# degleris1/CMF.jl

Hardware: AMD Instinct MI355X
Metric: MU iters/sec (convolutive NMF multiplicative update; achieved HBM GB/s in `hbm`) (higher is better)
Workload: dtype f32

## Files before the change

cmf.jl_amd/csrc/cmf_api.hip:

```cpp
#include "cmf_internal.h"

static void wb_free(cmf_handle_s *h);
static void wb_disarm(cmf_handle_s *h);

size_t n_partial(const cmf_handle_s *h)
{
    const CmfDims &d = h->d;
    size_t n = (size_t)(64 * h->conv_gx) * (size_t)std::max(h->conv_gy, h->conv_gy_ext);
    n = std::max(n, (size_t)(d.Np / 64) * d.KB * d.L);
    n = std::max(n, (size_t)((d.Tl + 63) / 64) * d.KB);
    n = std::max(n, 2 * (((size_t)d.Tl * d.K32 + 1023) / 1024));
    return n;
}

static int ensure_stage(cmf_handle_s *h, size_t elems)
{
    if (h->stage_elems >= elems) return CMF_OK;
    if (h->stage) HIPCHK(hipFree(h->stage));
    h->stage = nullptr;
    h->stage_elems = 0;
    HIPCHK(hipMalloc(&h->stage, elems * sizeof(double)));
    h->stage_elems = elems;
    return CMF_OK;
}
// ... 342 lines not shown
        TRYB(upload_cols(h, data, 0, Tl, true, true));
        if (h->halo_r > 0) TRYB(upload_cols(h, data + (size_t)Tl * N, Tl, h->halo_r, false, false));
        h->data_norm = std::sqrt(h->data_sumsq);
        h->have_data = true;
    }
#undef TRYB
#undef HIPB
    *out = h;
    return CMF_OK;
}


int launch_hxt_on(cmf_handle_s *h, const float *X0, const float *X1, int NpX, int nsrc, float *slabs, int nchunks, int chunk_len,
                         int main_rows, const float *left)
{
    ProfScope prof_(h, hxt_prof_class(h, X0, nsrc));
    const CmfDims &d = h->d;
    h->spec_gen = -1;
    HxtParams p;
    p.H = left ? left : h->H; p.X0 = X0; p.X1 = X1; p.slabs = slabs;
    p.Np = NpX; p.K32 = d.K32; p.KB = d.KB; p.PADL = d.PADL; p.L = d.L; p.Tl = main_rows >= 0 ? main_rows : d.Tl; p.chunk_len = chunk_len;
    p.G = h->hxt_groups; p.nsrc = nsrc;
    p.CG = hxt_cg(nchunks);
    dim3 grid((NpX / 128) * p.CG * h->hxt_groups, nchunks / p.CG, nsrc * d.KB), block(256);
    switch (h->hxt_LP) {
#define CASE(LP_) case LP_: hipLaunchKernelGGL((hxt_kernel<LP_>), grid, block, 0, h->stream, p); break;
        CASE(1) CASE(2) CASE(3) CASE(4) CASE(5) CASE(6) CASE(8)
#undef CASE
    default: return fail(CMF_ERR_STATE, "internal: bad hxt LP %d", h->hxt_LP);
    }
    for (int i = 0; i < 7; ++i)
        if (kHxtLP[i] == h->hxt_LP) h->launches[LA_HXT + i] += 1;
    h->launches[nsrc == 1 ? LA_HXT_NSRC1 : LA_HXT_NSRC2] += 1;
    h->launches[p.Tl < d.Tl ? LA_HXT_TAIL : LA_HXT_NO_TAIL] += 1;
    KCHK("hxt_kernel");
    return CMF_OK;
}

int launch_transconv(cmf_handle_s *h, int nsrc, const float *xt0, bool front_block)
{
    if (h->sk_tc) return launch_transconv_small(h, nsrc, xt0);
    ProfScope prof_(h, nsrc == 2 ? PROF_TRANSCONV : PROF_TRANSCONV_1);
    const CmfDims &d = h->d;
    TcParams p;
    p.Wn = h->Wn; p.XT0 = xt0 ? xt0 : h->XT; p.XT1 = h->estT; p.slabs = h->hslabs;
    p.NpW = d.Np;
    p.TP = d.TP; p.PADL = d.PADL; p.K32 = d.K32; p.KB = d.KB; p.L = d.L; p.Tl = d.Tl;
    p.nsrc = nsrc;
    p.C = (int)(rup(d.N, 8) / 8);
    p.W = nsrc == 2 ? h->tc_W : h->tc_W1;
    p.F = nsrc == 2 ? h->tc_S : h->tc_S1;
    p.wtab = h->tc_tab[nsrc == 2 ? 0 : 1];
    p.t_first = 0;
    p.slab_rows = d.Tl;
    if (front_block) {
        p.W = h->tc_W2; p.F = h->tc_S2; p.wtab = h->tc_tab[2];
        p.t_first = -128;
        p.slab_rows = d.Tl + 128;
// ... 9 lines not shown
    if (front_block) h->launches[LA_TC_FRONT] += 1;
    if (p.W >= 64 && p.W % 32 == 0) h->launches[LA_TC_XCD] += 1;
    KCHK("transconv_kernel");
    return CMF_OK;
}

int launch_slab_sum(cmf_handle_s *h, float *out, const float *in, int nslabs, size_t stride, bool take_carry,
                           CmfHxtTail tail)
{
    size_t n4 = stride / 4;
    int blocks = (int)std::min<size_t>(2048, (n4 + 255) / 256);
    CmfLossCarry carry{};
    if (take_carry && h->carry.partial) {
        carry = h->carry;
        h->carry = CmfLossCarry{};
    }
    hipLaunchKernelGGL(slab_sum_kernel, dim3(blocks + (carry.partial ? 1 : 0)), dim3(256), 0, h->stream, out, in, nslabs, stride, n4, carry, tail);
    h->launches[carry.partial ? LA_SLAB_SUM_CARRY : LA_SLAB_SUM] += 1;
    KCHK("slab_sum_kernel");
    return CMF_OK;
}

int hxt_contract(cmf_handle_s *h, const float *X0, const float *X1, int nsrc, float *out, bool take_carry, bool slabs_only, const float *left,
                 const float *leftT)
{
    const CmfDims &d = h->d;
    h->spec_gen = -1;
    if ((left == nullptr) != (leftT == nullptr)) return fail(CMF_ERR_STATE, "internal: a left operand of the C2 contraction needs both layouts");
    if (h->small_k) return hxt_contract_small(h, X0, X1, nsrc, out, take_carry, slabs_only, leftT);
    const int nch = nsrc == 2 ? h->hxt_nchunks : h->hxt_nchunks1, clen = nsrc == 2 ? h->hxt_chunk_len : h->hxt_chunk_len1;
    const int main_rows = nsrc == 2 ? h->hxt_main : h->hxt_main1;
    CMFTRY(launch_hxt_on(h, X0, X1, d.Np, nsrc, h->wslabs, nch, clen, main_rows, left));
    const CmfHxtTail tail{left ? left : h->H, X0, X1, d.Tl - main_rows, d.PADL + main_rows, d.L, d.K32, d.Np};
    return launch_slab_sum(h, out, h->wslabs, hxt_nslabs(nch), (size_t)nsrc * d.L * d.K32 * d.Np, take_carry, tail);
}

int read_scalar(cmf_handle_s *h, int slot, double *v)
{
    HIPCHK(hipMemcpyAsync(h->h_scalar + slot, h->d_scalar + slot, sizeof(double), hipMemcpyDeviceToHost, h->stream));
    HIPCHK(hipStreamSynchronize(h->stream));
    *v = h->h_scalar[slot];
    return CMF_OK;
}

static int check_ready(cmf_handle_s *h, bool need_data)
{
    if (!h) return fail(CMF_ERR_ARG, "handle is NULL");
    if (h->root_only) return fail(CMF_ERR_STATE, "this entry needs a single-GPU handle, not the front handle of a cmf_create_multi group");
    HIPCHK(hipSetDevice(h->device));
    if (!h->factors_set) return fail(CMF_ERR_STATE, "factors not set: call cmf_set_factors first");
    if (need_data && !h->have_data) return fail(CMF_ERR_STATE, "handle was created without data");
    return CMF_OK;
}

[[maybe_unused]] static void conv_kernel_order()
{
// ... 17 lines not shown
        CASE(CONV_ISM_PQ) CASE(CONV_ISM_PQ_T) CASE(CONV_ISM_LOSS) CASE(CONV_ISM_LOSS_PQ)
        CASE(CONV_BETAM_PQ) CASE(CONV_BETAM_PQ_T) CASE(CONV_BETAM_LOSS) CASE(CONV_BETAM_LOSS_PQ)
#undef CASE
    default: return fail(CMF_ERR_STATE, "internal: the MU rule launches no conv mode %d", conv_mode(family, base));
    }
}

static int mu_conv(cmf_handle_s *h, int base, float *out, int T_store, int gy)
{
    const MuForm &f = mu_form(h);
    return mu_launch_conv(h, base >= CONV_BASE_LOSS ? f.loss_family : f.store_family, base, out, T_store, gy, mu_buf(h, f.conv_data[base]));
}

static bool mu_est_current(const cmf_handle_s *h) { return h->reuse_est && h->est_kind == mu_est_kind(h); }

static bool w_speculated(cmf_handle_s *h)
{
    const bool hit = mu_fusions(h) && h->spec_gen >= 0 && h->spec_gen == h->est_gen && mu_est_current(h) && !h->carry.partial;
    h->spec_gen = -1;
    if (hit) h->spec_hits += 1;
    return hit;
}

static int mu_contract_c2(cmf_handle_s *h, bool slabs_only)
{
    const MuForm &f = mu_form(h);
    return hxt_contract(h, mu_buf(h, f.c2_src[0]), mu_buf(h, f.c2_src[1]), f.c2_nsrc, slabs_only ? nullptr : h->numden, !slabs_only, slabs_only);
}

static int mu_contract_w(cmf_handle_s *h, bool slabs_only)
{
    if (w_speculated(h)) return CMF_OK;
    if (!mu_est_current(h)) CMFTRY(mu_conv(h, CONV_BASE_STORE, h->est, h->d.Tl, h->conv_gy));
    set_est(h, mu_est_kind(h));
    return mu_contract_c2(h, slabs_only);
}

int w_partial_impl(cmf_handle_s *h) { return mu_contract_w(h, false); }

int w_partial_half_impl(cmf_handle_s *h, int den)
{
    const CmfDims &d = h->d;
    const size_t LKN = (size_t)d.L * d.K32 * d.Np;
    if (den) {
        if (!(h->reuse_est && h->est_kind == EST_CONV))
            CMFTRY(launch_conv<CONV_EST>(h, h->est, d.Tl, h->conv_gy));
        set_est(h, EST_CONV);
    }
    const float *src = den ? h->est : h->X;
    return hxt_contract(h, src, src, 1, h->numden + (den ? LKN : 0), den != 0);
}

int w_apply_impl(cmf_handle_s *h, double l1W, double l2W, const float *tail_src, float *tail_dst, int tail_n, const float *den)
{
    const CmfDims &d = h->d;
    dim3 grid(d.Np / 64, d.KB, d.L);
    if (!den) den = h->numden + (size_t)d.L * d.K32 * d.Np;
    const int step = mu_step_kind(h, mu_form(h));
    if (step == 2) {
        hipLaunchKernelGGL(w_update_pow_kernel, grid, dim3(256), 0, h->stream, h->Wt, h->Wn, h->numden, den, d.N, d.K, d.L, d.Np, d.K32, (float)l1W,
                           (float)(2.0 * l2W), tail_src, tail_dst, tail_n, h->mu_gamma);
        KCHK("w_update_pow_kernel");
        h->pow_launches += 1;
        set_est(h, EST_NONE);
        return CMF_OK;
    }
    const bool root = step == 1;
    hipLaunchKernelGGL(root ? w_update_sqrt_kernel : w_update_kernel, grid, dim3(256), 0, h->stream, h->Wt, h->Wn, h->numden, den,
                       d.N, d.K, d.L, d.Np, d.K32, (float)l1W, (float)(2.0 * l2W), tail_src, tail_dst, tail_n);
    KCHK(root ? "w_update_sqrt_kernel" : "w_update_kernel");
    set_est(h, EST_NONE);
    return CMF_OK;
}

static int w_phase_impl(cmf_handle_s *h, double l1W, double l2W)
{
    const CmfDims &d = h->d;
    const MuForm &f = mu_form(h);
    if (!(h->small_k && mu_fusions(h))) {
        CMFTRY(w_partial_impl(h));
        if (f.kl_den()) {
            hipLaunchKernelGGL(kl_hsum_kernel, dim3(d.K, KL_HCHUNKS), dim3(256), 0, h->stream, h->Ht, d.TP, d.PADL, d.Tl, h->kl_sums);
            KCHK("kl_hsum_kernel");
            hipLaunchKernelGGL(kl_den_w_kernel, dim3(d.L, d.K), dim3(256), 0, h->stream, h->Ht, h->kl_sums, h->numden + (size_t)d.L * d.K32 * d.Np, d.TP, d.PADL, d.Tl,
                               d.K32, d.Np);
            KCHK("kl_den_w_kernel");
        }
        if (!xo_active(h)) return w_apply_impl(h, l1W, l2W);
        CMFTRY(xo_fold_w(h));
        CMFTRY(w_apply_impl(h, l1W, l2W));
        xo_after_w(h);
        return CMF_OK;
    }
    CMFTRY(mu_contract_w(h, true));
    CmfLossCarry carry{};
    if (h->carry.partial) {
        carry = h->carry;
        h->carry = CmfLossCarry{};
    }
    hipLaunchKernelGGL(w_update_small_kernel, dim3(d.Np / 64 + 1, d.L, d.K), dim3(256), 0, h->stream, h->Wt, h->Wn, h->sk_tc ? h->sk_Wj : nullptr, h->sk_slabs,
                       h->sk_ngroups, d.N, d.K, d.L, d.Np, d.K32, h->sk_JP, h->sk3_Kg, h->sk3_GR, h->sk3_JP,
                       (float)l1W, (float)(2.0 * l2W), carry);
// ... 54 lines not shown
        KCHK("kl_den_h_kernel");
    }
    const int S = f.c3_nsrc == 2 ? h->tc_S : h->tc_S1;
    if (xo_active(h)) {
        const float *num = nullptr, *den = nullptr;
        CMFTRY(xo_h_tables(h, S, stride, f.h_num, f.h_den, &num, &den));
        return launch_h_update(h, mu_step_kind(h, f), num, (size_t)0, 1, den, (size_t)0, 1, d.Tl, d.PADL, l1H, l2H);
    }
    if (f.kl_den()) return launch_h_update(h, mu_step_kind(h, f), h->hslabs + f.h_num * TK, stride, S, h->kl_denH, (size_t)0, 1, d.Tl, d.PADL, l1H, l2H);
    return launch_h_update(h, mu_step_kind(h, f), h->hslabs + f.h_num * TK, stride, S, h->hslabs + f.h_den * TK, stride, S, d.Tl, d.PADL, l1H, l2H);
}

int launch_loss_conv(cmf_handle_s *h)
{
    if (!(h->reuse_est && !h->gram)) return mu_conv(h, CONV_BASE_LOSS, nullptr, h->d.Tl, h->conv_gy);
    CMFTRY(mu_conv(h, CONV_BASE_LOSS_STORE, h->est, h->d.Tl, h->conv_gy));
    set_est(h, mu_est_kind(h));
    return CMF_OK;
}

static int w_speculate(cmf_handle_s *h)
{
    if (!mu_est_current(h) || h->gram || h->group || h->carry.partial || !mu_fusions(h)) return CMF_OK;
    CMFTRY(mu_contract_c2(h, h->small_k));
    h->spec_gen = h->est_gen;
    return CMF_OK;
}

static int ensure_ring(cmf_handle_s *h)
{
    if (!h->h_ring) HIPCHK(hipHostMalloc(&h->h_ring, 3 * sizeof(double), hipHostMallocCoherent));
    return CMF_OK;
}

int loss_partial_impl(cmf_handle_s *h, double *sumsq, bool readback, double *host_out, bool speculate)
{
    volatile unsigned long long *word = nullptr;
    if (readback && !host_out) {
        CMFTRY(ensure_ring(h));
        host_out = h->h_ring + 2;
        word = reinterpret_cast<volatile unsigned long long *>(host_out);
        *word = CMF_SENTINEL64;
    }
    CMFTRY(launch_loss_conv(h));
    hipLaunchKernelGGL(loss_reduce_kernel, dim3(1), dim3(256), 0, h->stream, h->partial, h->conv_partials, h->d_scalar, host_out);
    KCHK("loss_reduce_kernel");
    if (speculate) CMFTRY(w_speculate(h));
// ... 423 lines not shown
}

int cmf_rccl_version(int *version, char *path, int64_t path_len)
{
    if (!version) return fail(CMF_ERR_ARG, "version is NULL");
    CMFTRY(rccl_load());
    RCCLCHK(g_rccl.GetVersion(version));
    if (path && path_len > 0) snprintf(path, (size_t)path_len, "%s", g_rccl.path.c_str());
    return CMF_OK;
}

int cmf_get_counter(cmf_handle h, const char *name, int64_t *value)
{
    if (!h || !name || !value) return fail(CMF_ERR_ARG, "NULL argument");
    if (std::strcmp(name, "hals_pipeline_reruns") == 0) { *value = h->hals_reruns; return CMF_OK; }
    if (std::strcmp(name, "plan:n_cu") == 0) {
        *value = (h->root_only && h->group && !h->group->sh.empty()) ? h->group->sh[0]->n_cu : h->n_cu;
        return CMF_OK;
    }
    if (std::strcmp(name, "writeback_calls") == 0) { *value = h->wb ? h->wb->armed_calls : 0; return CMF_OK; }
    if (std::strcmp(name, "speculated_contractions") == 0) { *value = h->spec_hits; return CMF_OK; }
    if (std::strcmp(name, "liveness_checks") == 0) { *value = g_liveness_checks.load(); return CMF_OK; }
    if (std::strcmp(name, "pow_update_launches") == 0) { *value = h->pow_launches; return CMF_OK; }
    if (std::strcmp(name, "xortho_launches") == 0) { *value = h->xo_launches; return CMF_OK; }
    if (admm_counter(h, name, value)) return CMF_OK;
    if (sep_counter(h, name, value)) return CMF_OK;
    if (anls_counter(h, name, value)) return CMF_OK;
    if (std::strcmp(name, "small_k_fused_h_updates") == 0) {
        *value = h->sk_fused_h;
        if (h->group)
            for (const cmf_handle_s *s : h->group->sh) *value += (s != h) ? s->sk_fused_h : 0;
        return CMF_OK;
    }
    if (std::strcmp(name, "writeback_overlapped") == 0) { *value = h->wb ? h->wb->hooked_calls : 0; return CMF_OK; }
    if (std::strncmp(name, "launches:", 9) == 0) {
        for (int c = 0; c < LA_NCLS; ++c)
            if (std::strcmp(name + 9, kLaunchNames[c]) == 0) {
                *value = h->launches[c];
                if (h->group)
                    for (const cmf_handle_s *s : h->group->sh) *value += (s != h) ? s->launches[c] : 0;
                return CMF_OK;
            }
        for (int c = 0; c < HL_NCLS; ++c)
            if (std::strcmp(name + 9, kHalsLaunchNames[c]) == 0) { *value = h->hals_launches[c]; return CMF_OK; }
        return fail(CMF_ERR_ARG, "unknown launch path '%s'", name + 9);
    }
    if (h->group) {
        cmf_group_s *g = h->group;
        if (std::strcmp(name, "allreduce_calls") == 0) { *value = g->n_allreduce; return CMF_OK; }
        if (std::strcmp(name, "allgather_calls") == 0) { *value = g->n_allgather; return CMF_OK; }
        if (std::strcmp(name, "halo_in_allreduce") == 0) { *value = (g->halo_opt && g->halo_can && !g->gram && g->nranks > 1) ? 1 : 0; return CMF_OK; }
        if (std::strcmp(name, "enqueue_ns") == 0) { *value = g->enqueue_ns; return CMF_OK; }
        if (std::strcmp(name, "enqueue_iters") == 0) { *value = g->enqueue_iters; return CMF_OK; }
        if (std::strcmp(name, "worker_ns") == 0) {
            int64_t m = 0;
            for (const auto &w : g->pool.w) m = std::max<int64_t>(m, w->busy_ns.load());
            *value = m;
            return CMF_OK;
        }
    }
    return fail(CMF_ERR_ARG, "unknown counter '%s'", name);
}

int cmf_set_stream(cmf_handle h, void *hip_stream)
{
    if (!h) return fail(CMF_ERR_ARG, "handle is NULL");
    if (h->group) return fail(CMF_ERR_STATE, "a group handle runs on its own per-device streams");
// ... 156 lines not shown
                HIPCHK(hipStreamSynchronize(h->stream));
                hals_plan(h);
            }
            return CMF_OK;
        }
        HIPCHK(hipSetDevice(h->device));
        HIPCHK(hipStreamSynchronize(h->stream));
        (name[5] == 'p' ? h->hals_opt_persist : name[5] == 'g' ? h->hals_opt_general : name[5] == 's' ? h->hals_opt_seg : h->hals_opt_lag) = value;
        if (h->hals_ready) hals_plan(h);
        return CMF_OK;
    }
    if (std::strcmp(name, "hals_prepare") == 0) {
        HIPCHK(hipSetDevice(h->device));
        return hals_ensure(h);
    }
    if (std::strcmp(name, "conv_split") == 0) {
        h->conv_split = value;
        set_est(h, EST_NONE);
        return CMF_OK;
    }
    if (std::strcmp(name, "small_k_fuse") == 0) {
        if (value < 0 || value > 2) return fail(CMF_ERR_ARG, "small_k_fuse must be 0, 1 or 2");
        h->sk_fuse = value;
        return CMF_OK;
    }
    if (std::strcmp(name, "small_k") == 0) {
        HIPCHK(hipSetDevice(h->device));
        HIPCHK(hipStreamSynchronize(h->stream));
        h->small_k = value != 0 && h->small_k_ok;
        h->sk_wj_gen = -1;
        h->sk_tc = h->small_k && (h->sk_tc_ok || value == 2);
        h->tc_S = h->sk_tc ? 2 * h->sk3_NS : h->tc_S_full;
        h->tc_S1 = h->sk_tc ? 2 * h->sk3_NS : h->tc_S1_full;
        set_est(h, EST_NONE);
        return CMF_OK;
    }
    if (std::strcmp(name, "reuse_est") == 0) {
        h->reuse_est = value != 0;
        set_est(h, EST_NONE);
        return CMF_OK;
    }
    if (std::strcmp(name, "speculate") == 0) {
        h->speculate = value != 0;
        h->spec_gen = -1;
        return CMF_OK;
    }
// ... 1168 lines not shown
```

cmf.jl_amd/csrc/cmf_internal.h:

```cpp
#pragma once
#pragma GCC visibility push(default)
#include "cmf_hip.h"
#pragma GCC visibility pop
#include "cmf_kernels.h"
#include "cmf_rng.h"
#include "cmf_writeback.h"

#include <algorithm>
#include <atomic>
#include <chrono>
#include <cmath>
#include <cstdarg>
#include <cstdio>
#include <cstring>
#include <functional>
#include <map>
#include <mutex>
#include <string>
#include <thread>
#include <vector>

inline thread_local std::string g_err;

static int fail(int code, const char *fmt, ...)
// ... 114 lines not shown
    "g_gemm_fold_small_kernel<1,RV>", "g_gemm_fold_small_kernel<2,RV>", "g_gemm_fold_small_kernel<3,RV>",
    "g_gemm_fold_small_kernel:split", "g_gemm_fold_small_kernel:fused_h",
    "gram_w_kernel", "gram_lag_corr", "gram_w_taps", "gram_h_mfma_kernel", "gram_h_kernel",
    "slab_sum_kernel", "slab_sum_kernel:carry", "slab_sum_small_kernel", "slab_sum_small_kernel:carry",
    "halo_pack2_kernel", "halo_unpack2_kernel", "halo_pack3_kernel", "halo_unpack3_kernel"};
static_assert(sizeof(kLaunchNames) / sizeof(kLaunchNames[0]) == LA_NCLS, "one name per launch path");

enum { HL_W_REG = 0,  HL_W_GEN = HL_W_REG + 10,
       HL_G_RESID, HL_G_DIFF, HL_G_SPEC, HL_W_SPECULATE,
       HL_P_INIT_DEN, HL_P_INIT_RESID, HL_P_INIT_SNAP,
       HL_PERSIST,  HL_PERSIST_CHASED = HL_PERSIST + 5, HL_CHASE, HL_CHASE_REST,
       HL_STAGE, HL_STAGE_LAG2, HL_STAGE_LAG3, HL_ROW_GEN, HL_PUSH_GEN, HL_NCLS };
static const int kHalsNQ[10] = {2, 4, 6, 8, 10, 12, 16, 20, 24, 32};
static const char *const kHalsLaunchNames[] = {
    "hals_w_sweep_reg_kernel<2>", "hals_w_sweep_reg_kernel<4>", "hals_w_sweep_reg_kernel<6>", "hals_w_sweep_reg_kernel<8>", "hals_w_sweep_reg_kernel<10>",
    "hals_w_sweep_reg_kernel<12>", "hals_w_sweep_reg_kernel<16>", "hals_w_sweep_reg_kernel<20>", "hals_w_sweep_reg_kernel<24>", "hals_w_sweep_reg_kernel<32>",
    "hals_w_sweep_gen_kernel",
    "hals_g:residual", "hals_g:difference", "hals_g:speculated", "hals_w_speculate",
    "hals_p_init_kernel:den", "hals_p_init_kernel:residual", "hals_p_init_kernel:snapshot",
    "hals_h_persist_kernel", "hals_h_persist_kernel:P1", "hals_h_persist_kernel:P2", "hals_h_persist_kernel:P3", "hals_h_persist_kernel:P4",
    "hals_h_persist_kernel:chased", "conv3_chase_kernel", "conv3_chase_kernel:rest",
    "hals_h_stage_kernel", "hals_h_stage_kernel:lag2", "hals_h_stage_kernel:lag3", "hals_h_row_gen_kernel", "hals_h_push_gen_kernel"};
static_assert(sizeof(kHalsLaunchNames) / sizeof(kHalsLaunchNames[0]) == HL_NCLS, "one name per HALS launch path");

#define CMF_DIV_BETA 3

enum EstKind : int {
    EST_NONE = 0,
    EST_CONV = 1,
    EST_RESID = 2,
    EST_RESID_MASKED = 3,
    EST_SIGN = 4,
    EST_SIGN_MASKED = 5,
    EST_MU_MASKED = 6,
    EST_KL_R = 7,
    EST_KL_R_MASKED = 8,
    EST_IS_PQ = 9,
    EST_BETA_PQ = 10,
    EST_IS_PQ_MASKED = 11,
    EST_BETA_PQ_MASKED = 12
};
static inline int pgd_est_kind(bool masked, bool loss_abs) { return EST_RESID + (masked ? 1 : 0) + (loss_abs ? 2 : 0); }
static_assert(EST_RESID_MASKED == EST_RESID + 1 && EST_SIGN == EST_RESID + 2 && EST_SIGN_MASKED == EST_RESID + 3, "pgd_est_kind");

struct cmf_handle_s {
    int device = 0;
// ... 88 lines not shown
    float mu_gamma = 1.f;
    int64_t pow_launches = 0;
    float beta_consts[11] = {};
    double data_sum = 0.0;
    int kl_mask = 0;
    float *kl_denH = nullptr;
    double *kl_sums = nullptr;
    int is_div = 0;
    int pq_mask = 0;
    float *Xs = nullptr, *XsT = nullptr;
    float *est2 = nullptr, *est2T = nullptr;

    double data_sumsq = 0.0, data_norm = 0.0;
    bool factors_set = false;
    bool have_data = false;
    bool reuse_est = true;
    int gram = 0;
    float *gram_numden_h = nullptr;
    bool prof = false;
    int prof_every = 1;
    int prof_seen[32] = {0};
    int64_t launches[LA_NCLS] = {0};
    int64_t hals_launches[HL_NCLS] = {0};
    struct ProfRec { hipEvent_t a, b; int cls; };
    unsigned prof_mask = 0;
    std::vector<ProfRec> prof_recs;
    std::vector<hipEvent_t> prof_pool;
    int est_kind = EST_NONE;
    void *arena = nullptr;
    size_t arena_bytes = 0;
    bool streams_may_hang = false;
    int64_t est_gen = 0;
    int64_t spec_gen = -1;
    int last_rule_call = 0;
    bool speculate = true;
    std::function<int()> after_reduce;
    int64_t hals_spec_gen = -1;
    int64_t spec_hits = 0;

    struct cmf_group_s *group = nullptr;
    bool root_only = false;
    hipStream_t own_comm_stream = nullptr, comm_stream = nullptr;
    hipEvent_t ev_c0 = nullptr, ev_c1 = nullptr;
    double *h_ring = nullptr;
    bool dev_stamps = false;
    CmfLossCarry carry{};
// ... 184 lines not shown
int gram_h_impl(cmf_handle_s *h, double l1H, double l2H, double *loss);
int pgd_w_impl(cmf_handle_s *h, double pen_sq, double pen_abs, int nonneg);
int pgd_h_impl(cmf_handle_s *h, double pen_sq, double pen_abs, int nonneg, double *loss);
int hals_h_impl(cmf_handle_s *h, double l1H, double l2H);
int hals_h_rerun(cmf_handle_s *h);
int gram_denom_h(cmf_handle_s *h, float *out);
int gram_tables(cmf_handle_s *h);
int group_pgd_w(cmf_handle_s *st, struct cmf_group_s *g, double pen_sq, double pen_abs, int nonneg);
int group_pgd_h(cmf_handle_s *st, struct cmf_group_s *g, double pen_sq, double pen_abs, int nonneg, double *loss);
int group_set_mask(struct cmf_group_s *g, const double *mask);
size_t n_partial(const cmf_handle_s *h);
hipError_t stream_acquire(int device, hipStream_t *s);
void plan(cmf_handle_s *h, int n_cu);
int upload_cols(cmf_handle_s *h, const double *src, int64_t tc, int64_t ncols, bool rows_layout, bool accumulate_sumsq,
                       float *rows_dst = nullptr, float *cols_dst = nullptr);
int create_impl(cmf_handle *out, int device, int64_t N, int64_t Tl, int64_t K, int64_t L,
                       const double *data, int64_t t_offset, int64_t T_global, bool sharded, long long n_cu_asked = kNoCuHook);
int launch_hxt_on(cmf_handle_s *h, const float *X0, const float *X1, int NpX, int nsrc, float *slabs, int nchunks, int chunk_len,
                         int main_rows = -1, const float *left = nullptr);
int launch_transconv(cmf_handle_s *h, int nsrc, const float *xt0 = nullptr, bool front_block = false);
int launch_slab_sum(cmf_handle_s *h, float *out, const float *in, int nslabs, size_t stride, bool take_carry = false,
                           CmfHxtTail tail = CmfHxtTail{nullptr, nullptr, nullptr, 0, 0, 0, 0, 0});
int hxt_contract(cmf_handle_s *h, const float *X0, const float *X1, int nsrc, float *out, bool take_carry = false, bool slabs_only = false,
                 const float *left = nullptr, const float *leftT = nullptr);
int hxt_contract_small(cmf_handle_s *h, const float *X0, const float *X1, int nsrc, float *out, bool take_carry, bool slabs_only,
                       const float *leftT = nullptr);
bool sk_can_fuse_h(const cmf_handle_s *h);
int launch_transconv_small(cmf_handle_s *h, int nsrc, const float *xt0, bool update_h = false, float l1 = 0.f, float two_l2 = 0.f);
int read_scalar(cmf_handle_s *h, int slot, double *v);
int w_partial_impl(cmf_handle_s *h);
int w_partial_half_impl(cmf_handle_s *h, int den);
int w_apply_impl(cmf_handle_s *h, double l1W, double l2W, const float *tail_src = nullptr, float *tail_dst = nullptr, int tail_n = 0,
                        const float *den = nullptr);
int h_update_impl(cmf_handle_s *h, double l1H, double l2H, bool front = false);
int launch_loss_conv(cmf_handle_s *h);
int loss_partial_impl(cmf_handle_s *h, double *sumsq, bool readback = true, double *host_out = nullptr, bool speculate = false);
int set_factors_impl(cmf_handle_s *h, const double *W, const double *H);
int get_factors_impl(cmf_handle_s *h, double *W, double *H);
int reduce_partials(cmf_handle_s *h, const double *partial, int n, int slot, double *v);
double wait_timeout_s();
int ensure_resid(cmf_handle_s *h, bool masked = false, bool loss_abs = false);
HalsRowParams hals_row_params(cmf_handle_s *h, double l1H, double l2H);
int hals_persist_launch(cmf_handle_s *h, const HalsRowParams &q, int debug = 0, bool clear_flags = true);
int pgd_unit_norm(cmf_handle_s *h, bool is_W);
int rccl_load();
int group_use(cmf_handle_s *s);
int group_join(cmf_group_s *g);
// ... 250 lines not shown
```

cmf.jl_amd/csrc/cmf_kernels.h:

```cpp
#pragma once
#include <hip/hip_runtime.h>
#include <type_traits>
#include <stdint.h>
#include "cmf_conv_modes.h"

typedef float f32x16 __attribute__((ext_vector_type(16)));
typedef float f32x4 __attribute__((ext_vector_type(4)));

#define CMF_EPS_F 2.220446049250313e-16f

struct CmfDims {
    int N, Tl, K, L;
    int Np;
    int KB;
    int K32;
    int PADL;
    int TP;
    int Lp;
};

__device__ __forceinline__ int cmf_crow(int r, int h) { return (r & 3) + 8 * (r >> 2) + 4 * h; }

__device__ __forceinline__ __amdgpu_buffer_rsrc_t cmf_rsrc(const void *base, size_t bytes)
{
// ... 1245 lines not shown
{
    __shared__ __attribute__((aligned(16))) float Hs[32 * CONV3_STRIDE];
    const int b = blockIdx.x;
    if (b < n_full) {
        const int n0 = (b % gx) * 64;
        if (n0 + 32 < p.N) conv3_tile<MODE, 2, NKP, PREQ>(p, Hs, (b / gx) * 64, n0, threadIdx.x, b);
        else conv3_tile<MODE, 1, NKP>(p, Hs, (b / gx) * 64, n0, threadIdx.x, b);
    } else {
        const int q = b - n_full, tile = n_full + (q >> 2), sub = q & 3;
        conv3_quarter<MODE, NKP>(p, Hs, (tile / gx) * 64 + (sub >> 1) * 32, (tile % gx) * 64 + (sub & 1) * 32, threadIdx.x, b);
    }
}

struct HxtParams {
    const float *H;
    const float *X0;
    const float *X1;
    float *slabs;
    int Np, K32, KB, PADL, L, Tl;
    int chunk_len;
    int G;
    int nsrc;
    int CG;
};

template <int LP>
__device__ __forceinline__ void hxt_load(float (&E)[LP], float (&O)[LP], float (&B)[LP], __amdgpu_buffer_rsrc_t hr,
                                         __amdgpu_buffer_rsrc_t xr, int hoff, int xoff, int row, int K32, int Np)
{
#pragma unroll
    for (int u = 0; u < LP; ++u) {
        E[u] = cmf_bload(hr, hoff, (row + 2 * u + 1) * K32 * 4);
        O[u] = cmf_bload(hr, hoff, (row + 2 * u) * K32 * 4);
        B[u] = cmf_bload(xr, xoff, (row + 2 * u) * Np * 4);
    }
}

template <int LP>
__device__ __forceinline__ void hxt_group(f32x16 (&acc)[2 * LP], const float (&Ep)[LP], const float (&Op)[LP],
                                          const float (&Ec)[LP], const float (&Oc)[LP], const float (&Bc)[LP])
{
#pragma unroll
    for (int u = 0; u < LP; ++u) {
#pragma unroll
        for (int m = 0; m < LP; ++m) {
            const float ae = (u - m >= 0) ? Ec[(u - m >= 0) ? (u - m) : 0] : Ep[(u - m >= 0) ? 0 : (u - m + LP)];
            const float ao = (u - m >= 0) ? Oc[(u - m >= 0) ? (u - m) : 0] : Op[(u - m >= 0) ? 0 : (u - m + LP)];
            acc[2 * m] = __builtin_amdgcn_mfma_f32_32x32x2f32(ae, Bc[u], acc[2 * m], 0, 0, 0);
            acc[2 * m + 1] = __builtin_amdgcn_mfma_f32_32x32x2f32(ao, Bc[u], acc[2 * m + 1], 0, 0, 0);
        }
    }
}

template <int LP>
__global__ __launch_bounds__(256, 1) void hxt_kernel(HxtParams p)
{
    const int lane = threadIdx.x & 63, wave = __builtin_amdgcn_readfirstlane(threadIdx.x >> 6);
    const int i = lane & 31, h = lane >> 5;
    int quad, lg;
    if ((gridDim.x / p.G) % 8 == 0) {
        lg = (blockIdx.x >> 3) % p.G;
        quad = (blockIdx.x & 7) + 8 * (blockIdx.x / (8 * p.G));
    } else {
        quad = blockIdx.x / p.G;
        lg = blockIdx.x % p.G;
    }
    const int CG = p.CG;
    const int cw = wave % CG, nw = wave / CG;
    const int nb = quad * (4 / CG) + nw;
    const int c = blockIdx.y * CG + cw;
    const int src = blockIdx.z % p.nsrc;
    const int kb = blockIdx.z / p.nsrc;
    const int lag0 = lg * 2 * LP;
    const int Np = p.Np, K32 = p.K32;
    const float *X = src ? p.X1 : p.X0;

    const int tc0 = c * p.chunk_len;
    int tc1 = tc0 + p.chunk_len;
    if (tc1 > p.Tl) tc1 = p.Tl;
    const int ngroups = (tc1 > tc0) ? (tc1 - tc0 + 6 * LP - 1) / (6 * LP) * 3 : 0;

    const float *hbase = p.H + (size_t)(p.PADL + tc0 - lag0 - 2 * LP - 1) * K32;
    const float *xbase = X + (size_t)(p.PADL + tc0 - 2 * LP) * Np;
    const __amdgpu_buffer_rsrc_t hr = cmf_rsrc(hbase, (size_t)(p.chunk_len + 12 * LP + 8) * K32 * 4);
    const __amdgpu_buffer_rsrc_t xr = cmf_rsrc(xbase, (size_t)(p.chunk_len + 12 * LP + 8) * Np * 4);
    const int hoff = (h * K32 + kb * 32 + i) * 4;
    const int xoff = (h * Np + nb * 32 + i) * 4;

    f32x16 acc[2 * LP];
#pragma unroll
    for (int a = 0; a < 2 * LP; ++a)
#pragma unroll
        for (int r = 0; r < 16; ++r) acc[a][r] = 0.f;

    float E0[LP], O0[LP], B0[LP], E1[LP], O1[LP], B1[LP], E2[LP], O2[LP], B2[LP];
    if (ngroups > 0) {
        hxt_load<LP>(E0, O0, B0, hr, xr, hoff, xoff, 0, K32, Np);
        hxt_load<LP>(E1, O1, B1, hr, xr, hoff, xoff, 2 * LP, K32, Np);
#define HXT_SCHED()                                                                   \
    do {                                                                              \
        constexpr int per = (2 * LP * LP >= 9 * LP) ? 2 : ((2 * LP * LP >= 6 * LP) ? 1 : 0);  \
        _Pragma("unroll") for (int q = 0; q < 3 * LP; ++q) {                          \
            __builtin_amdgcn_sched_group_barrier(0x020, 1, 0);                        \
            __builtin_amdgcn_sched_group_barrier(0x008, per, 0);                      \
        }                                                                             \
        __builtin_amdgcn_sched_group_barrier(0x008, 2 * LP * LP - per * 3 * LP, 0);   \
        __builtin_amdgcn_sched_barrier(0);                                            \
    } while (0)
        for (int g = 0; g < ngroups; g += 3) {
            const int g3 = (g + 3 < ngroups) ? g + 3 : g;
            hxt_load<LP>(E2, O2, B2, hr, xr, hoff, xoff, 2 * LP * (g + 2), K32, Np);
            hxt_group<LP>(acc, E0, O0, E1, O1, B1);
            HXT_SCHED();
            hxt_load<LP>(E0, O0, B0, hr, xr, hoff, xoff, 2 * LP * (g + 3), K32, Np);
            hxt_group<LP>(acc, E1, O1, E2, O2, B2);
            HXT_SCHED();
            hxt_load<LP>(E1, O1, B1, hr, xr, hoff, xoff, 2 * LP * (g3 + 1), K32, Np);
            hxt_group<LP>(acc, E2, O2, E0, O0, B0);
            HXT_SCHED();
        }
#undef HXT_SCHED
    }

    float *slab = p.slabs + (size_t)(blockIdx.y * p.nsrc + src) * p.L * K32 * Np;
    if (CG == 1) {
#pragma unroll
        for (int a = 0; a < 2 * LP; ++a) {
            int l = lag0 + a;
            if (l < p.L) {
#pragma unroll
                for (int r = 0; r < 16; ++r) {
                    int k = kb * 32 + cmf_crow(r, h);
                    slab[((size_t)l * K32 + k) * Np + nb * 32 + i] = acc[a][r];
                }
            }
        }
        return;
    }
    __shared__ float red[2][4][16][64];
#pragma unroll
    for (int a = 0; a < 2 * LP; ++a) {
        const int buf = a & 1;
#pragma unroll
        for (int r = 0; r < 16; ++r) red[buf][wave][r][lane] = acc[a][r];
        __syncthreads();
        const int l = lag0 + a;
        const int per = 16 / CG;
        for (int rr = 0; rr < per; ++rr) {
            const int r = cw * per + rr;
            float sum = red[buf][nw * CG][r][lane];
            for (int v = 1; v < CG; ++v) sum += red[buf][nw * CG + v][r][lane];
            const int k = kb * 32 + cmf_crow(r, h);
            if (l < p.L) slab[((size_t)l * K32 + k) * Np + nb * 32 + i] = sum;
        }
    }
}

struct TcParams {
    const float *Wn;
    const float *XT0;
    const float *XT1;
    float *slabs;
    int NpW;
    int TP, PADL, K32, KB, L, Tl;
    int nsrc;
    int C;
    int t_first;
    int slab_rows;
    int W;
    int F;
    const int4 *wtab;
};

#define TC_ROW 160
#define TC_CHUNK (8 * TC_ROW)

// ... 373 lines not shown
            const int n = (int)(e % tail.Np);
            const int k = (int)((e / tail.Np) % tail.K32);
            const int l = (int)((e / ((size_t)tail.Np * tail.K32)) % tail.L);
            const int src = (int)(e / ((size_t)tail.Np * tail.K32 * tail.L));
            const float *X = src ? tail.X1 : tail.X0;
            for (int r0 = 0; r0 < tail.rows; r0 += 6) {
                float hv[6];
                float4 xv[6];
#pragma unroll
                for (int u = 0; u < 6; ++u) {
                    const int t = tail.t0 + ((r0 + u < tail.rows) ? r0 + u : r0);
                    hv[u] = tail.H[(size_t)(t - l) * tail.K32 + k];
                    xv[u] = *reinterpret_cast<const float4 *>(X + (size_t)t * tail.Np + n);
                }
#pragma unroll
                for (int u = 0; u < 6; ++u)
                    if (r0 + u < tail.rows) {
                        a.x = fmaf(hv[u], xv[u].x, a.x); a.y = fmaf(hv[u], xv[u].y, a.y);
                        a.z = fmaf(hv[u], xv[u].z, a.z); a.w = fmaf(hv[u], xv[u].w, a.w);
                    }
            }
        }
        reinterpret_cast<float4 *>(out)[idx] = a;
    }
}

#define CMF_SENTINEL64 0xFFFFFFFFFFFFFFFFull
#define CMF_SENTINEL32 0xFFFFFFFFu
static __global__ __launch_bounds__(256) void loss_reduce_kernel(const double *partial, int n, double *out, double *host_out = nullptr)
{
    __shared__ double red[256];
    red[threadIdx.x] = cmf_thread_loss_sum(partial, n);
    __syncthreads();
    for (int off = 128; off > 0; off >>= 1) {
        if ((int)threadIdx.x < off) red[threadIdx.x] += red[threadIdx.x + off];
        __syncthreads();
    }
    if (threadIdx.x == 0) {
        *out = red[0];
        if (host_out) __hip_atomic_store(host_out, red[0], __ATOMIC_RELAXED, __HIP_MEMORY_SCOPE_SYSTEM);
    }
}



#define HALS_CORR_LPW 5
// ... 1858 lines not shown
```

Measured before the change: 187.8.

## Reduce HXT chunks in-block and fuse tail rows into W update

Adds an hxt_sum_kernel that runs every time-chunk of the W contraction inside one 512-thread block and reduces the chunks through shared memory. It writes the final numerator/denominator directly, which removes the slab buffer round trip and the separate slab_sum launch. The leftover time rows and the loss carry are deferred into a new w_update_tail_kernel that folds them into the multiplicative W update. It is enabled by default for the plain MU path (mu_tails=1). The trade-off is fewer blocks and reduced parallelism per launch, plus extra per-thread tail work inside the update kernel.

```diff
diff --git a/cmf.jl_amd/csrc/cmf_api.hip b/cmf.jl_amd/csrc/cmf_api.hip
--- a/cmf.jl_amd/csrc/cmf_api.hip
+++ b/cmf.jl_amd/csrc/cmf_api.hip
@@ -388,6 +388,7 @@
     p.Np = NpX; p.K32 = d.K32; p.KB = d.KB; p.PADL = d.PADL; p.L = d.L; p.Tl = main_rows >= 0 ? main_rows : d.Tl; p.chunk_len = chunk_len;
     p.G = h->hxt_groups; p.nsrc = nsrc;
     p.CG = hxt_cg(nchunks);
+    p.NBW = 0; p.CGS = 0;
     dim3 grid((NpX / 128) * p.CG * h->hxt_groups, nchunks / p.CG, nsrc * d.KB), block(256);
     switch (h->hxt_LP) {
 #define CASE(LP_) case LP_: hipLaunchKernelGGL((hxt_kernel<LP_>), grid, block, 0, h->stream, p); break;
@@ -400,6 +401,38 @@
     h->launches[nsrc == 1 ? LA_HXT_NSRC1 : LA_HXT_NSRC2] += 1;
     h->launches[p.Tl < d.Tl ? LA_HXT_TAIL : LA_HXT_NO_TAIL] += 1;
     KCHK("hxt_kernel");
+    return CMF_OK;
+}
+
+static int launch_hxt_sum(cmf_handle_s *h, const float *X0, const float *X1, int nsrc, float *out, int nchunks, int chunk_len, int main_rows, const float *left)
+{
+    if (nchunks == 1) {
+        h->tail_launches[TL_HXT_FINISHED] += 1;
+        return launch_hxt_on(h, X0, X1, h->d.Np, nsrc, out, 1, chunk_len, main_rows, left);
+    }
+    ProfScope prof_(h, hxt_prof_class(h, X0, nsrc));
+    const CmfDims &d = h->d;
+    h->spec_gen = -1;
+    HxtParams p;
+    p.H = left ? left : h->H; p.X0 = X0; p.X1 = X1; p.slabs = out;
+    p.Np = d.Np; p.K32 = d.K32; p.KB = d.KB; p.PADL = d.PADL; p.L = d.L; p.Tl = main_rows; p.chunk_len = chunk_len;
+    p.G = h->hxt_groups; p.nsrc = nsrc;
+    p.CG = nchunks;
+    p.NBW = nchunks <= 2 ? 4 : (nchunks <= 4 ? 2 : 1);
+    p.CGS = hxt_cg(nchunks);
+    dim3 grid((d.Np / 32 / p.NBW) * h->hxt_groups, 1, nsrc * d.KB), block(512);
+    switch (h->hxt_LP) {
+#define CASE(LP_) case LP_: hipLaunchKernelGGL((hxt_sum_kernel<LP_>), grid, block, 0, h->stream, p); break;
+        CASE(1) CASE(2) CASE(3) CASE(4) CASE(5)
+#undef CASE
+    default: return fail(CMF_ERR_STATE, "internal: hxt_sum_kernel has no LP %d", h->hxt_LP);
+    }
+    for (int i = 0; i < 7; ++i)
+        if (kHxtLP[i] == h->hxt_LP) h->launches[LA_HXT + i] += 1;
+    h->launches[nsrc == 1 ? LA_HXT_NSRC1 : LA_HXT_NSRC2] += 1;
+    h->launches[main_rows < d.Tl ? LA_HXT_TAIL : LA_HXT_NO_TAIL] += 1;
+    h->tail_launches[TL_HXT_SUM] += 1;
+    KCHK("hxt_sum_kernel");
     return CMF_OK;
 }
 
@@ -455,16 +488,22 @@
 }
 
 int hxt_contract(cmf_handle_s *h, const float *X0, const float *X1, int nsrc, float *out, bool take_carry, bool slabs_only, const float *left,
-                 const float *leftT)
+                 const float *leftT, bool defer_tail)
 {
     const CmfDims &d = h->d;
     h->spec_gen = -1;
+    h->w_tail.rows = 0;
     if ((left == nullptr) != (leftT == nullptr)) return fail(CMF_ERR_STATE, "internal: a left operand of the C2 contraction needs both layouts");
     if (h->small_k) return hxt_contract_small(h, X0, X1, nsrc, out, take_carry, slabs_only, leftT);
     const int nch = nsrc == 2 ? h->hxt_nchunks : h->hxt_nchunks1, clen = nsrc == 2 ? h->hxt_chunk_len : h->hxt_chunk_len1;
     const int main_rows = nsrc == 2 ? h->hxt_main : h->hxt_main1;
+    const CmfHxtTail tail{left ? left : h->H, X0, X1, d.Tl - main_rows, d.PADL + main_rows, d.L, d.K32, d.Np};
+    if (defer_tail && h->mu_tails && out && !slabs_only && nch <= 8 && h->hxt_LP <= 5) {
+        CMFTRY(launch_hxt_sum(h, X0, X1, nsrc, out, nch, clen, main_rows, left));
+        h->w_tail = tail;
+        return CMF_OK;
+    }
     CMFTRY(launch_hxt_on(h, X0, X1, d.Np, nsrc, h->wslabs, nch, clen, main_rows, left));
-    const CmfHxtTail tail{left ? left : h->H, X0, X1, d.Tl - main_rows, d.PADL + main_rows, d.L, d.K32, d.Np};
     return launch_slab_sum(h, out, h->wslabs, hxt_nslabs(nch), (size_t)nsrc * d.L * d.K32 * d.Np, take_carry, tail);
 }
 
@@ -528,18 +567,25 @@
     return hit;
 }
 
-static int mu_contract_c2(cmf_handle_s *h, bool slabs_only)
+static int mu_contract_c2(cmf_handle_s *h, bool slabs_only, bool defer_tail = false)
 {
     const MuForm &f = mu_form(h);
-    return hxt_contract(h, mu_buf(h, f.c2_src[0]), mu_buf(h, f.c2_src[1]), f.c2_nsrc, slabs_only ? nullptr : h->numden, !slabs_only, slabs_only);
-}
-
-static int mu_contract_w(cmf_handle_s *h, bool slabs_only)
+    return hxt_contract(h, mu_buf(h, f.c2_src[0]), mu_buf(h, f.c2_src[1]), f.c2_nsrc, slabs_only ? nullptr : h->numden, !slabs_only, slabs_only, nullptr, nullptr,
+                        defer_tail);
+}
+
+static bool mu_tails_w(cmf_handle_s *h)
+{
+    const MuForm &f = mu_form(h);
+    return h->mu_tails && !h->group && !h->sharded && !h->gram && !h->small_k && mu_fusions(h) && !f.kl_den() && mu_step_kind(h, f) == 0;
+}
+
+static int mu_contract_w(cmf_handle_s *h, bool slabs_only, bool defer_tail = false)
 {
     if (w_speculated(h)) return CMF_OK;
     if (!mu_est_current(h)) CMFTRY(mu_conv(h, CONV_BASE_STORE, h->est, h->d.Tl, h->conv_gy));
     set_est(h, mu_est_kind(h));
-    return mu_contract_c2(h, slabs_only);
+    return mu_contract_c2(h, slabs_only, defer_tail);
 }
 
 int w_partial_impl(cmf_handle_s *h) { return mu_contract_w(h, false); }
@@ -579,11 +625,35 @@
     return CMF_OK;
 }
 
+static int w_apply_tail(cmf_handle_s *h, double l1W, double l2W)
+{
+    const CmfDims &d = h->d;
+    const CmfHxtTail tail = h->w_tail;
+    h->w_tail.rows = 0;
+    if (tail.rows == 0 && !h->carry.partial) return w_apply_impl(h, l1W, l2W);
+    const CmfLossCarry carry = h->carry;
+    h->carry = CmfLossCarry{};
+    hipLaunchKernelGGL(w_update_tail_kernel, dim3(d.Np / 64 + (carry.partial ? 1 : 0), d.KB, d.L), dim3(256), 0, h->stream, h->Wt, h->Wn, h->numden,
+                       h->numden + (size_t)d.L * d.K32 * d.Np, d.N, d.K, d.L, d.Np, d.K32, (float)l1W, (float)(2.0 * l2W), carry, tail);
+    h->tail_launches[TL_W_TAIL] += 1;
+    if (carry.partial) h->tail_launches[TL_W_TAIL_CARRY] += 1;
+    if (tail.rows > 0) h->tail_launches[TL_W_TAIL_ROWS] += 1;
+    h->mu_tail_updates += 1;
+    KCHK("w_update_tail_kernel");
+    set_est(h, EST_NONE);
+    return CMF_OK;
+}
+
 static int w_phase_impl(cmf_handle_s *h, double l1W, double l2W)
 {
     const CmfDims &d = h->d;
     const MuForm &f = mu_form(h);
     if (!(h->small_k && mu_fusions(h))) {
+        if (mu_tails_w(h)) {
+            CMFTRY(mu_contract_w(h, false, true));
+            return w_apply_tail(h, l1W, l2W);
+        }
+        if (h->w_tail.rows > 0) h->spec_gen = -1;
         CMFTRY(w_partial_impl(h));
         if (f.kl_den()) {
             hipLaunchKernelGGL(kl_hsum_kernel, dim3(d.K, KL_HCHUNKS), dim3(256), 0, h->stream, h->Ht, d.TP, d.PADL, d.Tl, h->kl_sums);
@@ -684,7 +754,7 @@
 static int w_speculate(cmf_handle_s *h)
 {
     if (!mu_est_current(h) || h->gram || h->group || h->carry.partial || !mu_fusions(h)) return CMF_OK;
-    CMFTRY(mu_contract_c2(h, h->small_k));
+    CMFTRY(mu_contract_c2(h, h->small_k, mu_tails_w(h)));
     h->spec_gen = h->est_gen;
     return CMF_OK;
 }
@@ -1154,6 +1224,7 @@
     if (std::strcmp(name, "speculated_contractions") == 0) { *value = h->spec_hits; return CMF_OK; }
     if (std::strcmp(name, "liveness_checks") == 0) { *value = g_liveness_checks.load(); return CMF_OK; }
     if (std::strcmp(name, "pow_update_launches") == 0) { *value = h->pow_launches; return CMF_OK; }
+    if (std::strcmp(name, "mu_tail_updates") == 0) { *value = h->mu_tail_updates; return CMF_OK; }
     if (std::strcmp(name, "xortho_launches") == 0) { *value = h->xo_launches; return CMF_OK; }
     if (admm_counter(h, name, value)) return CMF_OK;
     if (sep_counter(h, name, value)) return CMF_OK;
@@ -1175,6 +1246,8 @@
             }
         for (int c = 0; c < HL_NCLS; ++c)
             if (std::strcmp(name + 9, kHalsLaunchNames[c]) == 0) { *value = h->hals_launches[c]; return CMF_OK; }
+        for (int c = 0; c < TL_NCLS; ++c)
+            if (std::strcmp(name + 9, kTailLaunchNames[c]) == 0) { *value = h->tail_launches[c]; return CMF_OK; }
         return fail(CMF_ERR_ARG, "unknown launch path '%s'", name + 9);
     }
     if (h->group) {
@@ -1377,6 +1450,12 @@
     if (std::strcmp(name, "small_k_fuse") == 0) {
         if (value < 0 || value > 2) return fail(CMF_ERR_ARG, "small_k_fuse must be 0, 1 or 2");
         h->sk_fuse = value;
+        return CMF_OK;
+    }
+    if (std::strcmp(name, "mu_tails") == 0) {
+        if (value != 0 && value != 1) return fail(CMF_ERR_ARG, "mu_tails must be 0 or 1");
+        h->mu_tails = value;
+        h->spec_gen = -1;
         return CMF_OK;
     }
     if (std::strcmp(name, "small_k") == 0) {
diff --git a/cmf.jl_amd/csrc/cmf_internal.h b/cmf.jl_amd/csrc/cmf_internal.h
--- a/cmf.jl_amd/csrc/cmf_internal.h
+++ b/cmf.jl_amd/csrc/cmf_internal.h
@@ -160,6 +160,11 @@
     "hals_h_persist_kernel:chased", "conv3_chase_kernel", "conv3_chase_kernel:rest",
     "hals_h_stage_kernel", "hals_h_stage_kernel:lag2", "hals_h_stage_kernel:lag3", "hals_h_row_gen_kernel", "hals_h_push_gen_kernel"};
 static_assert(sizeof(kHalsLaunchNames) / sizeof(kHalsLaunchNames[0]) == HL_NCLS, "one name per HALS launch path");
+
+enum { TL_HXT_SUM = 0, TL_HXT_FINISHED, TL_W_TAIL, TL_W_TAIL_CARRY, TL_W_TAIL_ROWS, TL_NCLS };
+static const char *const kTailLaunchNames[] = {"hxt_sum_kernel", "hxt_kernel:finished", "w_update_tail_kernel", "w_update_tail_kernel:carry",
+                                               "w_update_tail_kernel:rows"};
+static_assert(sizeof(kTailLaunchNames) / sizeof(kTailLaunchNames[0]) == TL_NCLS, "one name per mu_tails launch path");
 
 #define CMF_DIV_BETA 3
 
@@ -294,6 +299,10 @@
     int prof_seen[32] = {0};
     int64_t launches[LA_NCLS] = {0};
     int64_t hals_launches[HL_NCLS] = {0};
+    int64_t tail_launches[TL_NCLS] = {0};
+    int mu_tails = 1;
+    CmfHxtTail w_tail{nullptr, nullptr, nullptr, 0, 0, 0, 0, 0};
+    int64_t mu_tail_updates = 0;
     struct ProfRec { hipEvent_t a, b; int cls; };
     unsigned prof_mask = 0;
     std::vector<ProfRec> prof_recs;
@@ -524,7 +533,7 @@
 int launch_slab_sum(cmf_handle_s *h, float *out, const float *in, int nslabs, size_t stride, bool take_carry = false,
                            CmfHxtTail tail = CmfHxtTail{nullptr, nullptr, nullptr, 0, 0, 0, 0, 0});
 int hxt_contract(cmf_handle_s *h, const float *X0, const float *X1, int nsrc, float *out, bool take_carry = false, bool slabs_only = false,
-                 const float *left = nullptr, const float *leftT = nullptr);
+                 const float *left = nullptr, const float *leftT = nullptr, bool defer_tail = false);
 int hxt_contract_small(cmf_handle_s *h, const float *X0, const float *X1, int nsrc, float *out, bool take_carry, bool slabs_only,
                        const float *leftT = nullptr);
 bool sk_can_fuse_h(const cmf_handle_s *h);
diff --git a/cmf.jl_amd/csrc/cmf_kernels.h b/cmf.jl_amd/csrc/cmf_kernels.h
--- a/cmf.jl_amd/csrc/cmf_kernels.h
+++ b/cmf.jl_amd/csrc/cmf_kernels.h
@@ -1291,6 +1291,8 @@
     int G;
     int nsrc;
     int CG;
+    int NBW;
+    int CGS;
 };
 
 template <int LP>
@@ -1322,25 +1324,8 @@
 }
 
 template <int LP>
-__global__ __launch_bounds__(256, 1) void hxt_kernel(HxtParams p)
-{
-    const int lane = threadIdx.x & 63, wave = __builtin_amdgcn_readfirstlane(threadIdx.x >> 6);
-    const int i = lane & 31, h = lane >> 5;
-    int quad, lg;
-    if ((gridDim.x / p.G) % 8 == 0) {
-        lg = (blockIdx.x >> 3) % p.G;
-        quad = (blockIdx.x & 7) + 8 * (blockIdx.x / (8 * p.G));
-    } else {
-        quad = blockIdx.x / p.G;
-        lg = blockIdx.x % p.G;
-    }
-    const int CG = p.CG;
-    const int cw = wave % CG, nw = wave / CG;
-    const int nb = quad * (4 / CG) + nw;
-    const int c = blockIdx.y * CG + cw;
-    const int src = blockIdx.z % p.nsrc;
-    const int kb = blockIdx.z / p.nsrc;
-    const int lag0 = lg * 2 * LP;
+__device__ __forceinline__ void hxt_accumulate(const HxtParams &p, f32x16 (&acc)[2 * LP], int nb, int kb, int lag0, int src, int c, int i, int h)
+{
     const int Np = p.Np, K32 = p.K32;
     const float *X = src ? p.X1 : p.X0;
 
@@ -1356,7 +1341,6 @@
     const int hoff = (h * K32 + kb * 32 + i) * 4;
     const int xoff = (h * Np + nb * 32 + i) * 4;
 
-    f32x16 acc[2 * LP];
 #pragma unroll
     for (int a = 0; a < 2 * LP; ++a)
 #pragma unroll
@@ -1390,6 +1374,31 @@
         }
 #undef HXT_SCHED
     }
+}
+
+template <int LP>
+__global__ __launch_bounds__(256, 1) void hxt_kernel(HxtParams p)
+{
+    const int lane = threadIdx.x & 63, wave = __builtin_amdgcn_readfirstlane(threadIdx.x >> 6);
+    const int i = lane & 31, h = lane >> 5;
+    int quad, lg;
+    if ((gridDim.x / p.G) % 8 == 0) {
+        lg = (blockIdx.x >> 3) % p.G;
+        quad = (blockIdx.x & 7) + 8 * (blockIdx.x / (8 * p.G));
+    } else {
+        quad = blockIdx.x / p.G;
+        lg = blockIdx.x % p.G;
+    }
+    const int CG = p.CG;
+    const int cw = wave % CG, nw = wave / CG;
+    const int nb = quad * (4 / CG) + nw;
+    const int c = blockIdx.y * CG + cw;
+    const int src = blockIdx.z % p.nsrc;
+    const int kb = blockIdx.z / p.nsrc;
+    const int lag0 = lg * 2 * LP;
+    const int Np = p.Np, K32 = p.K32;
+    f32x16 acc[2 * LP];
+    hxt_accumulate<LP>(p, acc, nb, kb, lag0, src, c, i, h);
 
     float *slab = p.slabs + (size_t)(blockIdx.y * p.nsrc + src) * p.L * K32 * Np;
     if (CG == 1) {
@@ -1421,6 +1430,55 @@
             for (int v = 1; v < CG; ++v) sum += red[buf][nw * CG + v][r][lane];
             const int k = kb * 32 + cmf_crow(r, h);
             if (l < p.L) slab[((size_t)l * K32 + k) * Np + nb * 32 + i] = sum;
+        }
+    }
+}
+
+template <int LP>
+__global__ __launch_bounds__(512, 1) void hxt_sum_kernel(HxtParams p)
+{
+    const int lane = threadIdx.x & 63, wave = __builtin_amdgcn_readfirstlane(threadIdx.x >> 6);
+    const int i = lane & 31, h = lane >> 5;
+    int quad, lg;
+    if ((gridDim.x / p.G) % 8 == 0) {
+        lg = (blockIdx.x >> 3) % p.G;
+        quad = (blockIdx.x & 7) + 8 * (blockIdx.x / (8 * p.G));
+    } else {
+        quad = blockIdx.x / p.G;
+        lg = blockIdx.x % p.G;
+    }
+    const int CG = p.CG, NBW = p.NBW, CGS = p.CGS;
+    const int cw = wave % CG, nw = wave / CG;
+    const bool live = nw < NBW;
+    const int src = blockIdx.z % p.nsrc;
+    const int kb = blockIdx.z / p.nsrc;
+    const int lag0 = lg * 2 * LP;
+    const int Np = p.Np, K32 = p.K32;
+    f32x16 acc[2 * LP];
+    if (live) hxt_accumulate<LP>(p, acc, quad * NBW + nw, kb, lag0, src, cw, i, h);
+
+    float *out = p.slabs + (size_t)src * p.L * K32 * Np;
+    __shared__ float red[2][8][16][64];
+#pragma unroll
+    for (int a = 0; a < 2 * LP; ++a) {
+        const int buf = a & 1;
+        if (live) {
+#pragma unroll
+            for (int r = 0; r < 16; ++r) red[buf][wave][r][lane] = acc[a][r];
+        }
+        __syncthreads();
+        const int l = lag0 + a;
+        for (int j = 0; j < 2 * NBW; ++j) {
+            const int row = wave * 2 * NBW + j, nwj = row >> 4, r = row & 15;
+            const float *col = &red[buf][nwj * CG][r][lane];
+            float tot = 0.f;
+            for (int v0 = 0; v0 < CG; v0 += CGS) {
+                float sum = col[v0 * 1024];
+                for (int v = 1; v < CGS; ++v) sum += col[(v0 + v) * 1024];
+                tot = v0 ? tot + sum : sum;
+            }
+            const int k = kb * 32 + cmf_crow(r, h);
+            if (l < p.L) out[((size_t)l * K32 + k) * Np + (quad * NBW + nwj) * 32 + i] = tot;
         }
     }
 }
@@ -1840,6 +1898,66 @@
             }
         }
         reinterpret_cast<float4 *>(out)[idx] = a;
+    }
+}
+
+static __global__ __launch_bounds__(256) void w_update_tail_kernel(float *Wt, float *Wn, const float *num_p, const float *den_p, int N, int K, int L, int Np,
+                                                                   int K32, float l1, float two_l2, CmfLossCarry carry, CmfHxtTail tail)
+{
+    __shared__ float tile[32][65];
+    const int tid = threadIdx.x;
+    if ((int)blockIdx.x == Np / 64) {
+        if (blockIdx.y == 0 && blockIdx.z == 0) cmf_block_loss_reduce(carry);
+        return;
+    }
+    const int n0 = blockIdx.x * 64, kb = blockIdx.y, l = blockIdx.z;
+    {
+        const int nn = tid & 63, n = n0 + nn, k0 = kb * 32 + (tid >> 6);
+        float num[8], den[8], w[8];
+#pragma unroll
+        for (int q = 0; q < 8; ++q) {
+            const size_t idx = ((size_t)l * K32 + k0 + 4 * q) * Np + n;
+            num[q] = num_p[idx];
+            den[q] = den_p[idx];
+            w[q] = Wt[idx];
+        }
+        for (int r0 = 0; r0 < tail.rows; r0 += 6) {
+            float x0[6], x1[6], hv[6][8];
+#pragma unroll
+            for (int u = 0; u < 6; ++u) {
+                const int t = tail.t0 + ((r0 + u < tail.rows) ? r0 + u : r0);
+                x0[u] = tail.X0[(size_t)t * Np + n];
+                x1[u] = tail.X1[(size_t)t * Np + n];
+#pragma unroll
+                for (int q = 0; q < 8; ++q) hv[u][q] = tail.H[(size_t)(t - l) * K32 + k0 + 4 * q];
+            }
+#pragma unroll
+            for (int u = 0; u < 6; ++u)
+                if (r0 + u < tail.rows) {
+#pragma unroll
+                    for (int q = 0; q < 8; ++q) {
+                        num[q] = fmaf(hv[u][q], x0[u], num[q]);
+                        den[q] = fmaf(hv[u][q], x1[u], den[q]);
+                    }
+                }
+        }
+#pragma unroll
+        for (int q = 0; q < 8; ++q) {
+            const int kk = q * 4 + (tid >> 6), k = kb * 32 + kk;
+            const size_t idx = ((size_t)l * K32 + k) * Np + n;
+            const float wn = (k < K && n < N) ? cmf_mu(w[q], num[q], den[q], l1, two_l2) : 0.f;
+            Wt[idx] = wn;
+            tile[kk][nn] = wn;
+        }
+    }
+    __syncthreads();
+    {
+        const int kk = tid & 31;
+#pragma unroll
+        for (int q = 0; q < 8; ++q) {
+            const int nn = q * 8 + (tid >> 5);
+            Wn[((size_t)l * Np + n0 + nn) * K32 + kb * 32 + kk] = tile[kk][nn];
+        }
     }
 }
 
```

Result: no change. 188.7 (median of 6 runs) (+0.4%).
